# andrewli77/combinatorial-rl-tasks

Hardware: NVIDIA B200
Metric: env_steps_per_sec (higher is better)
Workload: dtype f32

## Files before the change

combinatorial_rl_tasks_b200/csrc/crl_kernels.cu:

```cuda
#include <cuda_runtime.h>

#include <atomic>
#include <stdint.h>
#include <stdio.h>
#include <string.h>

#include "../../include/crl_b200.h"
#include "crl_core.cuh"

namespace crl {

#ifndef CRL_THREADS
#define CRL_THREADS 64
#endif
constexpr int kThreads = CRL_THREADS;
constexpr unsigned kFull = 0xffffffffu;

struct KParams {
  int B, num_steps, frameskip, max_cd, seed_mode, env_offset;
  long long min_seed, max_seed;
  double thresh2;
  float r2_guard;
  double bonus_per_step;
  double beta_a, beta_b;
  float robot_keepout, zone_keepout, extent;
  unsigned flags;
  DivConst div_steps, div_cd;
  unsigned long long action_seed, step_index;
  float4* pose;
  float4* aux;
  float2* zone_xy;
  uint32_t* zone_tmax;
  uint2* cooldown;
  long long* seed;
  uint32_t* episode;
  float4* origin;
  double* counters;
  float2* next_zone_xy;
  uint32_t* next_task;
  float4* next_origin;
  long long* next_seed;
  uint32_t* next_ready;
  uint32_t* stamp;
  uint32_t* act_count;
  const uint32_t* epoch;
  uint32_t round;
  uint32_t* row_list;
  float* zone_obs_host;
  unsigned long long* result_dev;
  int32_t* goal;
  const float2* bank_zone_xy;
  const float4* bank_origin;
  const uint32_t* bank_task;
  const float4* fixed;
  uint32_t init_hi;
  uint32_t walled;
  const float2* actions;
  float4* obs;
  float* zone_obs;
  unsigned long long* result;
  float* shaped;
  const uint8_t* mask;
};

constexpr uint32_t kParBit = 0x8000u, kHiMask = 0x7fffu;

template <int TASK>
struct ZoneDim { static constexpr int Z = (TASK == CRL_TASK_TSP) ? 6 : 7; };

#ifndef CRL_REGS_N15
#define CRL_REGS_N15 112
#endif
template <int N>
struct MaxRegs { static constexpr int v = N > 8 ? CRL_REGS_N15 : 80; };

template <int N>
struct Env {
  Body b;
  float ep_return;
  int steps;
  uint32_t hi;
  float2 zone[N];
  uint32_t tmax[(N + 1) / 2];
  uint2 cd;
};

__device__ __forceinline__ uint32_t cd_get(const uint2& cd, int i) {
  const uint32_t w = i < 4 ? cd.x : cd.y;
  return (w >> (8 * (i & 3))) & 0xffu;
}
__device__ __forceinline__ void cd_set(uint2& cd, int i, uint32_t v) {
  uint32_t& w = i < 4 ? cd.x : cd.y;
  const int sh = 8 * (i & 3);
  w = (w & ~(0xffu << sh)) | (v << sh);
}
__device__ __forceinline__ uint32_t cd_dec4(uint32_t w) {
  const uint32_t nz = (((w & 0x7f7f7f7fu) + 0x7f7f7f7fu) | w) >> 7 & 0x01010101u;
  return w - nz;
}


__device__ __forceinline__ U4 draw(long long seed, uint32_t c0, uint32_t c1, uint32_t c2, uint32_t tag) {
  U4 ctr{c0, c1, c2, tag};
  return philox4x32(ctr, (uint32_t)(unsigned long long)seed, (uint32_t)((unsigned long long)seed >> 32));
}

__device__ double gamma_mt(long long seed, double a, uint32_t zone, uint32_t which) {
  const double d = a - 1.0 / 3.0, c = 1.0 / sqrt(9.0 * d);
  for (uint32_t it = 0;; ++it) {
    const U4 r0 = draw(seed, it, zone, which, kTagTask);
    const U4 r1 = draw(seed, it, zone, which + 2u, kTagTask);
    const double u1 = u01d(r0.x, r0.y), u2 = u01d(r0.z, r0.w), u3 = u01d(r1.x, r1.y);
    const double x = sqrt(-2.0 * log(u1)) * cos(2.0 * kPi * u2);
    double v = 1.0 + c * x;
    if (v <= 0.0) continue;
    v = v * v * v;
    if (log(u3) < 0.5 * x * x + d - d * v + d * log(v) || it > 64u) return d * v;
  }
}

__device__ double gamma_half_integer(long long seed, int k, uint32_t zone, uint32_t which) {
  const int m = k >> 1;
  double prod = 1.0, U = 1.0, V = 0.0;
  const int n_u = m + ((k & 1) ? 2 : 0);
  for (int j = 0; j < n_u; j += 2) {
    const U4 r = draw(seed, (uint32_t)(j >> 1), zone, which, kTagTask);
    const double ua = u01d(r.x, r.y), ub = u01d(r.z, r.w);
    if (j < m) prod *= ua; else if (j == m) U = ua; else V = ua;
    if (j + 1 < m) prod *= ub; else if (j + 1 == m) U = ub; else if (j + 1 < n_u) V = ub;
  }
  double g = -log(prod);
  if (k & 1) {
    const double c = cos(2.0 * kPi * V);
    g += -log(U) * (c * c);
  }
  return g;
}

CRL_HD int half_integer_shape(double a) {
  const double t = 2.0 * a;
  const int k = (int)t;
  return ((double)k == t && k >= 1 && k <= 16) ? k : 0;
}

__device__ double gamma_draw(long long seed, double a, uint32_t zone, uint32_t which) {
  const int k = half_integer_shape(a);
  return k ? gamma_half_integer(seed, k, zone, which) : gamma_mt(seed, a, zone, which);
}

__device__ uint32_t colour_draw(long long seed, uint32_t zone) {
  uint32_t c = 3u;
  for (uint32_t it = 0; c == 3u && it < 64u; ++it) {
    const U4 r = draw(seed, it, zone, 0u, kTagTask);
    uint32_t bits = r.x;
    for (int q = 0; q < 16 && c == 3u; ++q, bits >>= 2) c = bits & 3u;
  }
  return c == 3u ? 0u : c;
}

template <int N, bool FIXED>
__device__ void warp_layout(const KParams& p, long long seed, float2* placed, int lane) {
  const float ext = p.extent;
  constexpr int NP = (N + 2) / 2;
#pragma unroll 1
  for (uint32_t attempt = 0; attempt < 10000u; ++attempt) {
    bool ok_layout = true;
#pragma unroll 1
    for (int k = 0; k <= N && ok_layout; ++k) {
      const float keep = k == 0 ? p.robot_keepout : p.zone_keepout;
      float lo_x = -ext + keep, lo_y = lo_x, span = (ext - keep) - lo_x;
      if (FIXED && p.fixed) {
        const float4 fx = p.fixed[k];
        if (fx.w == 1.f || fx.w == 3.f) { lo_x = fx.x; lo_y = fx.y; span = 0.f; }
      }
      float4 pl[NP];
#pragma unroll
      for (int q2 = 0; q2 < NP; ++q2) pl[q2] = reinterpret_cast<const float4*>(placed)[q2];
      bool found = false;
#pragma unroll 1
      for (int base = 0; base < 100 && !found; base += 32) {
        const int j = base + lane;
        const U4 r = draw(seed, (uint32_t)(j >> 1), (uint32_t)k, attempt, kTagLayout);
        const float x = __fadd_rn(lo_x, __fmul_rn(span, u01((j & 1) ? r.z : r.x)));
        const float y = __fadd_rn(lo_y, __fmul_rn(span, u01((j & 1) ? r.w : r.y)));
        bool valid = j < 100;
#pragma unroll
        for (int q = 0; q < N; ++q) {
          const float ox = (q & 1) ? pl[q >> 1].z : pl[q >> 1].x;
          const float oy = (q & 1) ? pl[q >> 1].w : pl[q >> 1].y;
          const float need = __fadd_rn(q == 0 ? p.robot_keepout : p.zone_keepout, keep);
          const float dx = __fsub_rn(x, ox), dy = __fsub_rn(y, oy);
          const float d2 = __fmaf_rn(dy, dy, __fmul_rn(dx, dx));
          valid = valid && (q >= k || d2 >= __fmul_rn(need, need));
        }
        const unsigned m = __ballot_sync(kFull, valid);
        if (m) {
          const int wlane = __ffs(m) - 1;
          const float wx = __shfl_sync(kFull, x, wlane), wy = __shfl_sync(kFull, y, wlane);
          if (lane == 0) placed[k] = make_float2(wx, wy);
          found = true;
        }
      }
      __syncwarp();
      ok_layout = found;
    }
    if (ok_layout) return;
  }
}

__device__ __forceinline__ long long choose_seed(const KParams& p, int e, uint32_t episode, uint32_t ahead = 0u) {
  if (p.seed_mode != CRL_SEED_FIXED_RANGE) return p.seed[e] + (long long)ahead;
  const unsigned long long span = (unsigned long long)(p.max_seed - p.min_seed) + 1ull;
  const U4 r = draw((long long)(p.env_offset + e), episode + ahead, 0u, 0u, kTagSeed);
  const unsigned long long v = ((unsigned long long)r.x << 32) | r.y;
  return p.min_seed + (long long)(span ? (v % span) : v);
}

template <int TASK, int N, bool FIXED>
__device__ void warp_generate(const KParams& p, long long chosen, float2* placed, int lane,
                              uint32_t& my_draw, float& rot0) {
  my_draw = 0u;
  if (TASK == CRL_TASK_TTSP && lane < N) {
    const double ga = gamma_draw(chosen, p.beta_a, (uint32_t)lane, 0u);
    const double gb = gamma_draw(chosen, p.beta_b, (uint32_t)lane, 1u);
    const int t = (int)((ga / (ga + gb)) * (double)p.num_steps);
    my_draw = (uint32_t)min(max(t, 0), 65535);
  }
  if (TASK == CRL_TASK_CM && lane < N) my_draw = colour_draw(chosen, (uint32_t)lane);
  warp_layout<N, FIXED>(p, chosen + 1, placed, lane);
  const U4 rr = draw(chosen + 1, 0u, 0u, 0u, kTagRot);
  rot0 = __fmul_rn(6.2831855f, u01(rr.x));
  if (FIXED && p.fixed) { const float4 f0 = p.fixed[0]; if (f0.w >= 2.f) rot0 = f0.z; }
  __syncwarp();
}

constexpr uint32_t kSlotEmpty = 0u, kSlotLayoutDone = 2u, kSlotClaimed = 3u, kSlotReady = 16u;

__device__ __forceinline__ uint32_t ld_acquire_u32(const uint32_t* p) {
  uint32_t v;
  asm volatile("ld.acquire.gpu.global.u32 %0, [%1];" : "=r"(v) : "l"(p) : "memory");
  return v;
}
// ... 383 lines not shown
    } else {
      const bool v = (env.hi >> i) & 1u;
      r = v ? 1.f : 0.f; g = 1.f; b = v ? 0.f : 1.f;
    }
    float* z = row + i * Z;
    if (Z == 6) {
      reinterpret_cast<float2*>(z)[0] = make_float2(env.zone[i].x * third, env.zone[i].y * third);
      reinterpret_cast<float2*>(z)[1] = make_float2(r, g);
      reinterpret_cast<float2*>(z)[2] = make_float2(b, 0.25f);
    } else {
      z[0] = env.zone[i].x * third; z[1] = env.zone[i].y * third;
      z[2] = r; z[3] = g; z[4] = b; z[5] = 0.25f;
      if (TASK == CRL_TASK_TTSP) {
        const bool v = (env.hi >> i) & 1u;
        const int tm = (int)((env.tmax[i >> 1] >> (16 * (i & 1))) & 0xffffu);
        z[6] = v ? 1.0f : div_const((float)(tm - env.steps), p.div_steps);
      } else {
        z[6] = div_const((float)cd_get(env.cd, i), p.div_cd);
      }
    }
  }
}

template <int TASK, int N>
__device__ __forceinline__ void zone_obs_issue(const KParams& p, float* stage, int lane, int env0, int max_rows) {
  constexpr int ROW = N * ZoneDim<TASK>::Z;
  const int n_valid = max(0, min(max_rows, p.B - env0));
  const uint32_t bytes = (uint32_t)n_valid * ROW * 4u;
  float* gdst = p.zone_obs + (size_t)env0 * ROW;
  if ((bytes & 15u) == 0u) {
    asm volatile("fence.proxy.async.shared::cta;" ::: "memory");
    __syncwarp();
    if (lane == 0 && n_valid > 0) {
      const uint32_t saddr = (uint32_t)__cvta_generic_to_shared(stage);
      asm volatile("cp.async.bulk.global.shared::cta.bulk_group [%0], [%1], %2;"
                   :: "l"(gdst), "r"(saddr), "r"(bytes) : "memory");
      asm volatile("cp.async.bulk.commit_group;" ::: "memory");
    }
  } else {
    __syncwarp();
    for (int i = lane; i < n_valid * ROW; i += 32) gdst[i] = stage[i];
  }
}

template <int TASK, int N>
__device__ __forceinline__ void zone_obs_send(const KParams& p, const Env<N>& env, bool valid,
                                              float* stage, int lane, int warp_env0, bool zero_row = false) {
  constexpr int ROW = N * ZoneDim<TASK>::Z;
  if (valid) zone_row<TASK, N>(p, env, stage + lane * ROW);
  if (zero_row) {
    for (int k = 0; k < ROW; ++k) stage[lane * ROW + k] = 0.f;
  }
  zone_obs_issue<TASK, N>(p, stage, lane, warp_env0, 32);
}

template <int TASK, int N>
__device__ __noinline__ void send_rows(const KParams& p, float* out, const float* stage, unsigned mask, int lane,
                                       int warp_env0) {
  constexpr int Z = ZoneDim<TASK>::Z, ROW = N * Z;
  if (TASK == CRL_TASK_TTSP && (p.flags & CRL_STEP_HOST_PLANES)) {
    const size_t plane = (size_t)p.B * N;
    const int n_valid = max(0, min(32, p.B - warp_env0));
    float* tl = out + 6 * plane + (size_t)warp_env0 * N;
    for (int i = lane; i < n_valid * N; i += 32) tl[i] = stage[(i / N) * ROW + (i % N) * Z + 6];
    while (mask) {
      const int src = __ffs(mask) - 1;
      mask &= mask - 1u;
      const float* row = stage + src * ROW;
      float* dst = out + (size_t)(warp_env0 + src) * N;
      for (int i = lane; i < 6 * N; i += 32) dst[(size_t)(i / N) * plane + (i % N)] = row[(i % N) * Z + (i / N)];
    }
    return;
  }
  while (mask) {
    const int src = __ffs(mask) - 1;
    mask &= mask - 1u;
    float* dst = out + (size_t)(warp_env0 + src) * ROW;
    const float* row = stage + src * ROW;
    for (int i = lane; i < ROW; i += 32) dst[i] = row[i];
  }
}

template <int TASK, int N>
__device__ __forceinline__ bool zone_obs_step(const KParams& p, const Env<N>& env, float* stage, int lane, int warp_env0,
                                              unsigned changed) {
  constexpr int ROW = N * ZoneDim<TASK>::Z;
  const int n_valid = max(0, min(32, p.B - warp_env0));
  const unsigned all = n_valid >= 32 ? kFull : (1u << n_valid) - 1u;
  const unsigned m = (p.flags & CRL_STEP_ZONE_OBS_DELTA) ? changed : all;
  if ((m >> lane) & 1u) zone_row<TASK, N>(p, env, stage + lane * ROW);
  if (m != all) return false;
  zone_obs_issue<TASK, N>(p, stage, lane, warp_env0, 32);
  return true;
}

__device__ __forceinline__ void zone_obs_wait(int lane) {
  if (lane == 0) asm volatile("cp.async.bulk.wait_group.read 0;" ::: "memory");
}

constexpr int kParkedSteps = 0xffff;
__device__ void obs_rows_bulk(float4* obs, int B, float4 row0, float4 row1, bool valid, float* stage, int lane, int warp_env0);

template <int TASK, int N>
__device__ __forceinline__ void store_state_obs(const KParams& p, const Env<N>& env, int e, float c, float s,
                                                bool park = false) {
  p.pose[e] = make_float4(env.b.X, env.b.Y, env.b.phi, env.b.vx);
  p.aux[e] = make_float4(env.b.vy, env.b.w, env.ep_return,
                         __int_as_float((int)((uint32_t)(park ? kParkedSteps : env.steps) | (env.hi << 16))));
  if (TASK == CRL_TASK_CM) p.cooldown[e] = env.cd;
  const float remaining = div_const((float)(p.num_steps - env.steps), p.div_steps);
  p.obs[2 * (size_t)e] = make_float4(remaining, env.b.X * (1.0f / 3.0f), env.b.Y * (1.0f / 3.0f), c);
  p.obs[2 * (size_t)e + 1] = make_float4(s, env.b.vx * (1.0f / 1.5f), env.b.vy * (1.0f / 1.5f),
                                         env.b.w * (1.0f / 3.0f));
}

template <int TASK, int N>
__device__ __forceinline__ void store_state_obs_host(const KParams& p, const Env<N>& env, bool valid, int e, float c, float s,
                                                     float* stage, int lane, int warp_env0) {
  if (valid) {
    p.pose[e] = make_float4(env.b.X, env.b.Y, env.b.phi, env.b.vx);
    p.aux[e] = make_float4(env.b.vy, env.b.w, env.ep_return, __int_as_float((int)((uint32_t)env.steps | (env.hi << 16))));
    if (TASK == CRL_TASK_CM) p.cooldown[e] = env.cd;
  }
  const float remaining = div_const((float)(p.num_steps - env.steps), p.div_steps);
  obs_rows_bulk(p.obs, p.B, make_float4(remaining, env.b.X * (1.0f / 3.0f), env.b.Y * (1.0f / 3.0f), c),
                make_float4(s, env.b.vx * (1.0f / 1.5f), env.b.vy * (1.0f / 1.5f), env.b.w * (1.0f / 3.0f)), valid, stage, lane,
                warp_env0);
}

__device__ __noinline__ void obs_rows_bulk(float4* obs, int B, float4 row0, float4 row1, bool valid, float* stage, int lane,
                                           int warp_env0) {
  if (lane == 0) asm volatile("cp.async.bulk.wait_group.read 0;" ::: "memory");
  __syncwarp();
  if (valid) {
    float4* row = reinterpret_cast<float4*>(stage) + 2 * lane;
    row[0] = row0;
    row[1] = row1;
  }
  asm volatile("fence.proxy.async.shared::cta;" ::: "memory");
  __syncwarp();
  const int n_valid = max(0, min(32, B - warp_env0));
  if (lane == 0 && n_valid > 0) {
    const uint32_t saddr = (uint32_t)__cvta_generic_to_shared(stage);
    float4* gdst = obs + 2 * (size_t)warp_env0;
    asm volatile("cp.async.bulk.global.shared::cta.bulk_group [%0], [%1], %2;"
                 :: "l"(gdst), "r"(saddr), "r"((uint32_t)n_valid * 32u) : "memory");
    asm volatile("cp.async.bulk.commit_group;" ::: "memory");
  }
}

template <int TASK, int N>
__device__ __forceinline__ void load_env(const KParams& p, int e, Env<N>& env) {
  const float4 ps = p.pose[e];
  const float4 ax = p.aux[e];
#pragma unroll
  for (int i = 0; i < N; ++i) env.zone[i] = p.zone_xy[(size_t)i * p.B + e];
  if (TASK == CRL_TASK_TTSP) {
#pragma unroll
    for (int j = 0; j < (N + 1) / 2; ++j) env.tmax[j] = p.zone_tmax[(size_t)j * p.B + e];
  }
  if (TASK == CRL_TASK_CM) env.cd = p.cooldown[e];
  env.b.X = ps.x; env.b.Y = ps.y; env.b.phi = ps.z; env.b.vx = ps.w;
  env.b.vy = ax.x; env.b.w = ax.y; env.ep_return = ax.z;
  const uint32_t bits = (uint32_t)__float_as_int(ax.w);
  env.steps = (int)(bits & 0xffffu);
  env.hi = bits >> 16;
}

__device__ __forceinline__ double dist_np(float X, float Y, float zx, float zy) {
  const double dx = (double)zx - (double)X, dy = (double)zy - (double)Y;
  return __dsqrt_rn(__dadd_rn(__dmul_rn(dx, dx), __dmul_rn(dy, dy)));
}

__device__ __forceinline__ uint32_t chain_ticket(const KParams& p, int w, int lane) {
  uint32_t t = 0u;
  if (lane == 0 && w < (p.B + 31) / 32) t = atomicAdd(p.stamp + w, 1u);
  return t;
}

__device__ __forceinline__ void chain_wait(const KParams& p, int w, int lane, uint32_t ticket) {
  if (lane == 0 && w < (p.B + 31) / 32) {
    const uint32_t* fin = p.stamp + (p.B + 31) / 32 + w;
    uint32_t polls = 0;
    while (ld_acquire_u32(fin) != ticket) {
      __nanosleep(64);
      if (++polls > (1u << 22)) { atomicAdd(p.counters + 7, 1.0); break; }
    }
  }
  __syncwarp();
}

__device__ __forceinline__ void chain_release(const KParams& p, int w, int lane, uint32_t ticket) {
  __syncwarp();
  if (lane == 0) {
    asm volatile("cp.async.bulk.wait_group 0;" ::: "memory");
    if (w < (p.B + 31) / 32) st_release_u32(p.stamp + (p.B + 31) / 32 + w, ticket + 1u);
  }
}

template <int TASK, int N, bool EXT, bool FIXED = false>
__global__ void __maxnreg__(MaxRegs<N>::v) step_kernel(const __grid_constant__ KParams p) {
  constexpr int ROW = N * ZoneDim<TASK>::Z;
  extern __shared__ __align__(128) float smem[];
  const int lane = threadIdx.x & 31, warp = threadIdx.x >> 5;
  const int e = blockIdx.x * kThreads + threadIdx.x;
  const int warp_env0 = blockIdx.x * kThreads + warp * 32;
  const bool valid = e < p.B;
  float* stage = smem + warp * (32 * ROW);
  uint32_t ticket = 0u;
  const bool ticketed = (p.flags & (CRL_STEP_CHAINED | CRL_STEP_CHAIN_START)) != 0u;
  if (ticketed) {
    ticket = chain_ticket(p, warp_env0 >> 5, lane);
    asm volatile("griddepcontrol.launch_dependents;" :: "r"(ticket) : "memory");
  } else {
    asm volatile("griddepcontrol.launch_dependents;" ::: "memory");
  }
  if (p.flags & CRL_STEP_CHAINED) {
    chain_wait(p, warp_env0 >> 5, lane, ticket);
  } else {
    asm volatile("griddepcontrol.wait;" ::: "memory");
  }

  uint32_t act_base = 0u;
  uint32_t* act_cnt = nullptr;
  if (!p.actions && (p.flags & CRL_STEP_ACTION_COUNTER) && lane == 0 && warp_env0 < p.B) {
    act_cnt = p.act_count + (warp_env0 >> 5);
    act_base = ld_relaxed_u32(act_cnt);
  }
  Env<N> env;
  float2 act = make_float2(0.f, 0.f);
  if (valid) load_env<TASK, N>(p, e, env);
  if (!p.actions && (p.flags & CRL_STEP_ACTION_COUNTER)) {
    if (act_cnt) *act_cnt = act_base + 1u;
    act_base = __shfl_sync(kFull, act_base, 0);
  }
  if (valid) {
    if (p.actions) {
      act = p.actions[e];
    } else {
      const unsigned ge = (unsigned)(p.env_offset + e);
      const unsigned long long si = p.step_index + act_base;
      U4 ctr{ge, (uint32_t)si, (uint32_t)(si >> 32), kTagAction};
      const U4 r = philox4x32(ctr, (uint32_t)p.action_seed, (uint32_t)(p.action_seed >> 32));
      act = make_float2(2.f * u01(r.x) - 1.f, 2.f * u01(r.y) - 1.f);
    }
  } else {
    env.b = Body{0.f, 0.f, 0.f, 0.f, 0.f, 0.f};
    env.ep_return = 0.f; env.steps = 0; env.hi = 0u; env.cd = make_uint2(0u, 0u);
#pragma unroll
    for (int i = 0; i < N; ++i) env.zone[i] = make_float2(1e9f, 1e9f);
#pragma unroll
    for (int j = 0; j < (N + 1) / 2; ++j) env.tmax[j] = 0xffffffffu;
  }

  const bool parked = EXT && (p.flags & CRL_STEP_WAIT) && valid && env.steps == kParkedSteps;
  const bool live = valid && !parked;
  const bool revive = EXT && parked && (p.flags & CRL_STEP_AUTO_RESET);
  const bool goals = EXT && (p.flags & CRL_STEP_GOALS);
  int goal_zone = -1;
  float gzx = 0.f, gzy = 0.f;
  double dist_before = 0.0;
  Body old_b = env.b;
  bool reached = false, park_now = false;
  if (goals && live) {
    goal_zone = p.goal[e];
    if (goal_zone >= 0) {
#pragma unroll
      for (int j = 0; j < N; ++j) if (j == goal_zone) { gzx = env.zone[j].x; gzy = env.zone[j].y; }
      dist_before = dist_np(env.b.X, env.b.Y, gzx, gzy);
    }
  }
  int fired_out = -1;
  __shared__ unsigned s_rows_mask[kThreads / 32];
  const bool some_rows = p.zone_obs_host || (p.flags & CRL_STEP_ZONE_OBS_DELTA);
  if (some_rows && lane == 0) s_rows_mask[warp] = 0u;
  bool fresh = false;
  if (!(p.flags & CRL_STEP_PHYSICS_ONLY)) {
    bool row_changed = TASK == CRL_TASK_TTSP && !(p.flags & CRL_STEP_HOST_PLANES);
    if (TASK == CRL_TASK_CM) {
      row_changed = (env.cd.x | env.cd.y) != 0u;
      env.cd.x = cd_dec4(env.cd.x); env.cd.y = cd_dec4(env.cd.y);
    }
    uint32_t cand = 0u;
#pragma unroll
    for (int i = 0; i < N; ++i)
      if (near_zone(env.b.X, env.b.Y, env.zone[i].x, env.zone[i].y, p.r2_guard)) cand |= 1u << i;
    if (TASK == CRL_TASK_CM) {
      if (cand) {
#pragma unroll
        for (int i = 0; i < N; ++i) if (cd_get(env.cd, i) != 0u) cand &= ~(1u << i);
      }
    } else {
      cand &= ~env.hi;
    }
    int fired = -1;
    while (cand) {
      const int i = __ffs(cand) - 1;
      cand &= cand - 1u;
      float zx = 0.f, zy = 0.f;
#pragma unroll
      for (int j = 0; j < N; ++j) if (j == i) { zx = env.zone[j].x; zy = env.zone[j].y; }
      if (inside_zone(env.b.X, env.b.Y, zx, zy, p.thresh2)) { fired = i; break; }
    }
    int event = 0;
    if (fired >= 0) {
      if (TASK == CRL_TASK_CM) {
        const int old_dist = hamming(env.hi, N);
        const uint32_t col = (env.hi >> (2 * fired)) & 3u;
        const uint32_t nxt = col == 2u ? 0u : col + 1u;
        env.hi = (env.hi & ~(3u << (2 * fired))) | (nxt << (2 * fired));
        cd_set(env.cd, fired, (uint32_t)p.max_cd);
        event = old_dist - hamming(env.hi, N);
      } else {
        env.hi |= 1u << fired;
        event = 1;
      }
    }
    bool goal;
    if (TASK == CRL_TASK_CM) {
      constexpr uint32_t kOnes = ((1u << (2 * N)) - 1u) & 0x55555555u;
      const uint32_t col = env.hi & kHiMask;
      goal = col == 0u || col == kOnes || col == 2u * kOnes;
    } else {
      goal = (env.hi & kHiMask) == ((1u << N) - 1u);
    }
    bool done = false;
    float reward = (float)event;
    if (goal) {
      reward = (float)((double)event + (double)(p.num_steps - env.steps) * p.bonus_per_step);
      done = true;
    }
    env.steps = min(env.steps + 1, kParkedSteps - 1);
    if (env.steps >= p.num_steps) done = true;
    if (TASK == CRL_TASK_TTSP && !done) {
#pragma unroll
      for (int i = 0; i < N; ++i) {
        const int tm = (int)((env.tmax[i >> 1] >> (16 * (i & 1))) & 0xffffu);
        if (!((env.hi >> i) & 1u) && env.steps >= tm) done = true;
      }
    }
    env.ep_return += reward;
    done = done && live;
    goal = goal && live;
    if (EXT) {
      fired_out = fired;
      reached = goals && fired >= 0 && fired == goal_zone;
      park_now = (p.flags & CRL_STEP_WAIT) && done && !(p.flags & CRL_STEP_AUTO_RESET);
      if (parked) { reward = 0.f; event = 0; }
    }
    if (p.flags & (CRL_STEP_TRACK_ROWS | CRL_STEP_ZONE_OBS_DELTA)) {
      const bool ch = (live && (row_changed || fired >= 0 || (done && (p.flags & CRL_STEP_AUTO_RESET)))) || parked;
      const unsigned cm = __ballot_sync(kFull, ch);
      if (some_rows && lane == 0) s_rows_mask[warp] = cm;
      if ((p.flags & CRL_STEP_TRACK_ROWS) && cm && lane == 0) atomicAdd(p.row_list, __popc(cm));
    }
    bool res_moved = false;
    if (valid) {
      const bool need_next = goals && live && (reached || done || goal_zone < 0);
      const unsigned long long word = (unsigned long long)__float_as_uint(reward) |
          ((unsigned long long)((done || parked) ? 1u : 0u) << 32) | ((unsigned long long)(goal ? 1u : 0u) << 40) |
          ((unsigned long long)(uint8_t)(int8_t)event << 48) | ((unsigned long long)(need_next ? 1u : 0u) << 56);
      if (p.result_dev) {
        const unsigned long long prev = p.result_dev[e];
        p.result_dev[e] = word;
        if (prev != word) { p.result[e] = word; res_moved = true; }
      } else {
        p.result[e] = word;
      }
      if (EXT && goals && live && need_next && goal_zone >= 0) p.goal[e] = -1;
    }
    if (p.result_dev) {
      const unsigned mm = __ballot_sync(kFull, res_moved);
      if (mm && lane == 0) atomicAdd(p.row_list + 1, (uint32_t)__popc(mm));
    }
    const unsigned dm = __ballot_sync(kFull, done);
    const unsigned rm = EXT ? __ballot_sync(kFull, done || revive) : dm;
    if (rm) {
      float ret = done ? env.ep_return : 0.f;
      float len = done ? (float)env.steps : 0.f;
      const unsigned gm = __ballot_sync(kFull, goal);
#pragma unroll
      for (int o = 16; o > 0; o >>= 1) {
        ret += __shfl_xor_sync(kFull, ret, o);
        len += __shfl_xor_sync(kFull, len, o);
      }
      if (lane == 0 && dm) {
        atomicAdd(p.counters + 0, (double)ret);
        atomicAdd(p.counters + 1, (double)__popc(dm));
        atomicAdd(p.counters + 2, (double)__popc(gm));
        atomicAdd(p.counters + 3, (double)len);
      }
      if (p.flags & CRL_STEP_AUTO_RESET) {
        fresh = done || revive;
        const uint32_t par_in = env.hi >> 15;
        bool served = false;
        if (fresh) served = reset_from_slot<TASK, N>(p, e, env);
        const unsigned sm = __ballot_sync(kFull, served);
        if (lane == 0 && sm) atomicAdd(p.counters + 4, (double)__popc(sm));
        const unsigned left = rm & ~sm;
        if (left) {
          Env<N> next = env;
          warp_reset<TASK, N, FIXED>(p, left, lane, e, reinterpret_cast<float2*>(stage), par_in, next);
          env = next;
        }
      }
    }
  }
  float c, s;
  if (!EXT) {
    unsigned rows = 0u;
    if (some_rows) {
      __syncwarp();
      rows = s_rows_mask[warp];
    }
    if (!(p.flags & CRL_STEP_NO_ZONE_OBS) && zone_obs_step<TASK, N>(p, env, stage, lane, warp_env0, rows) && !p.zone_obs_host)
      rows = 0u;
    if (rows || p.zone_obs_host) {
      __syncwarp();
      send_rows<TASK, N>(p, p.zone_obs_host ? p.zone_obs_host : p.zone_obs, stage, rows, lane, warp_env0);
    }
    if (fresh) {
      sincosf(env.b.phi, &s, &c);
    } else {
      substeps(env.b, act.x, act.y, p.frameskip, c, s);
      env.b.phi = wrap_pi(env.b.phi);
    }
    if (p.zone_obs_host) {
      store_state_obs_host<TASK, N>(p, env, valid, e, c, s, stage, lane, warp_env0);
    } else if (valid) {
      store_state_obs<TASK, N>(p, env, e, c, s);
    }
  } else {
    if (!(p.flags & CRL_STEP_NO_ZONE_OBS))
      zone_obs_send<TASK, N>(p, env, live || revive, stage, lane, warp_env0, parked && !revive);
    if (p.zone_obs_host) send_rows<TASK, N>(p, p.zone_obs_host, stage, s_rows_mask[warp], lane, warp_env0);
    Body pb = fresh ? old_b : env.b;
    if (p.walled) substeps<CRL_CONTACT_MODEL, true>(pb, act.x, act.y, p.frameskip, c, s, p.extent);
    else substeps(pb, act.x, act.y, p.frameskip, c, s);
    if (fresh) {
      sincosf(env.b.phi, &s, &c);
    } else {
      env.b = pb;
      env.b.phi = wrap_pi(env.b.phi);
    }
    if (goals && live) {
      double shaped = 0.0;
      if (goal_zone >= 0 && !reached) {
        shaped = dist_before - dist_np(pb.X, pb.Y, gzx, gzy);
        if (TASK == CRL_TASK_CM && fired_out >= 0) shaped -= 1.0;
      }
      p.shaped[e] = (float)shaped;
    }
    if (parked && goals) p.shaped[e] = 0.f;
    if (parked && !revive) {
      p.obs[2 * (size_t)e] = make_float4(0.f, 0.f, 0.f, 0.f);
      p.obs[2 * (size_t)e + 1] = make_float4(0.f, 0.f, 0.f, 0.f);
    } else if (valid) {
      store_state_obs<TASK, N>(p, env, e, c, s, park_now);
    }
  }
  if (ticketed) {
    chain_release(p, warp_env0 >> 5, lane, ticket);
  } else {
    zone_obs_wait(lane);
  }
}

template <int TASK, int N>
__global__ void __launch_bounds__(kThreads) reset_kernel(const __grid_constant__ KParams p) {
  constexpr int ROW = N * ZoneDim<TASK>::Z;
  extern __shared__ __align__(128) float smem[];
  const int lane = threadIdx.x & 31, warp = threadIdx.x >> 5;
  const int e = blockIdx.x * kThreads + threadIdx.x;
  const int warp_env0 = blockIdx.x * kThreads + warp * 32;
  const bool valid = e < p.B;
  float* stage = smem + warp * (32 * ROW);
  Env<N> env;
  if (valid) load_env<TASK, N>(p, e, env);
  const bool want = valid && (p.mask == nullptr || p.mask[e] != 0);
  const unsigned m = __ballot_sync(kFull, want);
  if (m) warp_reset<TASK, N, true, true>(p, m, lane, e, reinterpret_cast<float2*>(stage), 0u, env);
  float c = 1.f, s = 0.f;
  if (valid) sincosf(env.b.phi, &s, &c);
  zone_obs_send<TASK, N>(p, env, valid, stage, lane, warp_env0);
  if (want) store_state_obs<TASK, N>(p, env, e, c, s);
  zone_obs_wait(lane);
}

struct LayoutParams {
  const double* xy0; const double* rot0; const double* zone_xy;
  const int32_t* zone_max_steps; const int32_t* colours; const int32_t* env_ids; int n;
};

template <int TASK, int N>
__global__ void reset_from_layout_kernel(const KParams p, const LayoutParams L) {
  constexpr int ROW = N * ZoneDim<TASK>::Z;
  const int i = blockIdx.x * blockDim.x + threadIdx.x;
  if (i >= L.n) return;
  const int e = L.env_ids ? L.env_ids[i] : i;
  if (e < 0 || e >= p.B) return;
  Env<N> env;
  const float rot0 = (float)L.rot0[i];
  env.b = Body{(float)L.xy0[2 * i], (float)L.xy0[2 * i + 1], wrap_pi(rot0), 0.f, 0.f, 0.f};
  env.ep_return = 0.f; env.steps = 0; env.hi = TASK == CRL_TASK_CM ? 0u : p.init_hi; env.cd = make_uint2(0u, 0u);
#pragma unroll
  for (int j = 0; j < (N + 1) / 2; ++j) env.tmax[j] = 0u;
#pragma unroll
  for (int z = 0; z < N; ++z) {
    env.zone[z] = make_float2((float)L.zone_xy[((size_t)i * N + z) * 2], (float)L.zone_xy[((size_t)i * N + z) * 2 + 1]);
    p.zone_xy[(size_t)z * p.B + e] = env.zone[z];
    if (TASK == CRL_TASK_TTSP) {
      const uint32_t t = (uint32_t)min(max(L.zone_max_steps[(size_t)i * N + z], 0), 65535);
      env.tmax[z >> 1] |= t << (16 * (z & 1));
    }
    if (TASK == CRL_TASK_CM) env.hi |= ((uint32_t)L.colours[(size_t)i * N + z] & 3u) << (2 * z);
  }
  if (TASK == CRL_TASK_TTSP) {
#pragma unroll
    for (int j = 0; j < (N + 1) / 2; ++j) p.zone_tmax[(size_t)j * p.B + e] = env.tmax[j];
  }
  const uint32_t episode = p.episode[e] + 1u;
  p.episode[e] = episode;
  if (p.goal) p.goal[e] = -1;
  p.origin[e] = make_float4(env.b.X, env.b.Y, rot0, 0.f);
  p.pose[e] = make_float4(env.b.X, env.b.Y, env.b.phi, 0.f);
  p.aux[e] = make_float4(0.f, 0.f, 0.f, __int_as_float((int)((env.hi << 16) | ((episode & 1u) << 31))));
  if (TASK == CRL_TASK_CM) p.cooldown[e] = env.cd;
  float c, s;
  sincosf(env.b.phi, &s, &c);
  p.obs[2 * (size_t)e] = make_float4(1.0f, env.b.X * (1.0f / 3.0f), env.b.Y * (1.0f / 3.0f), c);
  p.obs[2 * (size_t)e + 1] = make_float4(s, 0.f, 0.f, 0.f);
  __align__(16) float row[ROW];
  zone_row<TASK, N>(p, env, row);
  float* g = p.zone_obs + (size_t)e * ROW;
#pragma unroll
  for (int k = 0; k < ROW; ++k) g[k] = row[k];
}

__global__ void set_qpos_qvel_kernel(const KParams p, const double* qpos, const double* qvel,
                                     const int32_t* env_ids, int n) {
  const int i = blockIdx.x * blockDim.x + threadIdx.x;
  if (i >= n) return;
  const int e = env_ids ? env_ids[i] : i;
  if (e < 0 || e >= p.B) return;
  const float4 o = p.origin[e];
  const double c0 = cos((double)o.z), s0 = sin((double)o.z);
// ... 219 lines not shown
  for (int i = 0; i < used; ++i)
    if (slots[i].d == d && slots[i].lo == n_lo && slots[i].hi == n_hi) return slots[i].k;
  const DivConst k = make_div_const(d, n_lo, n_hi);
  if (used < 8) slots[used++] = Slot{d, n_lo, n_hi, k};
  return k;
}

static int fill_params(const CrlConfig* c, const CrlState* st, const CrlOut* out, KParams& p) {
  int rc = check_config(c);
  if (rc) return rc;
  if (!st || !st->pose || !st->aux || !st->zone_xy || !st->seed || !st->episode || !st->origin || !st->counters)
    return CRL_ERR_NULL;
  if (c->task == CRL_TASK_TTSP && !st->zone_tmax) return CRL_ERR_NULL;
  if (c->task == CRL_TASK_CM && !st->cooldown) return CRL_ERR_NULL;
  if (!aligned16(st->pose) || !aligned16(st->aux) || !aligned16(st->zone_xy) || !aligned16(st->origin))
    return CRL_ERR_ALIGN;
  memset(&p, 0, sizeof(p));
  p.B = c->num_envs; p.num_steps = c->num_steps; p.frameskip = c->frameskip; p.max_cd = c->max_cooldown;
  p.seed_mode = c->seed_mode; p.env_offset = c->env_offset; p.min_seed = c->min_seed; p.max_seed = c->max_seed;
  p.thresh2 = sqrt_threshold(c->zone_size);
  p.r2_guard = (float)(c->zone_size * c->zone_size * 1.001 + 1e-5);
  p.bonus_per_step = c->time_saved_reward;
  p.beta_a = c->beta_a; p.beta_b = c->beta_b;
  p.div_steps = cached_div_const(c->num_steps, -65535, 65535);
  p.div_cd = cached_div_const(c->max_cooldown > 0 ? c->max_cooldown : 1, 0, 255);
  if (!p.div_steps.exact || !p.div_cd.exact) return CRL_ERR_CONFIG;
  p.robot_keepout = (float)c->robot_keepout; p.zone_keepout = (float)c->zone_keepout; p.extent = (float)c->extent;
  p.pose = reinterpret_cast<float4*>(st->pose); p.aux = reinterpret_cast<float4*>(st->aux);
  p.zone_xy = reinterpret_cast<float2*>(st->zone_xy); p.zone_tmax = st->zone_tmax;
  p.cooldown = reinterpret_cast<uint2*>(st->cooldown);
  p.seed = reinterpret_cast<long long*>(st->seed); p.episode = st->episode;
  p.origin = reinterpret_cast<float4*>(st->origin); p.counters = st->counters;
  if (st->next_ready) {
    if (!st->next_zone_xy || !st->next_origin || !st->next_seed || (c->task != CRL_TASK_TSP && !st->next_task))
      return CRL_ERR_NULL;
    if (!aligned16(st->next_origin) || !aligned16(st->next_zone_xy)) return CRL_ERR_ALIGN;
    p.next_zone_xy = reinterpret_cast<float2*>(st->next_zone_xy); p.next_task = st->next_task;
    p.next_origin = reinterpret_cast<float4*>(st->next_origin);
    p.next_seed = reinterpret_cast<long long*>(st->next_seed); p.next_ready = st->next_ready;
  }
  if (st->fixed_layout) {
    if (!aligned16(st->fixed_layout)) return CRL_ERR_ALIGN;
    p.fixed = reinterpret_cast<const float4*>(st->fixed_layout);
  }
  p.init_hi = c->task == CRL_TASK_CM ? 0u : c->initial_visited;
  p.walled = c->walled;
  p.stamp = st->stamp;
  p.act_count = st->stamp ? st->stamp + 2 * (size_t)((c->num_envs + 31) / 32) : nullptr;
  p.epoch = st->prefetch_epoch;
  if (p.next_ready && !p.epoch) return CRL_ERR_NULL;
  p.row_list = st->row_list;
  p.goal = st->goal;
  if (st->bank_zone_xy || st->bank_origin || st->bank_task) {
    if (!st->bank_zone_xy || !st->bank_origin || (c->task != CRL_TASK_TSP && !st->bank_task)) return CRL_ERR_NULL;
    if (c->max_seed < c->min_seed) return CRL_ERR_CONFIG;
    if (!aligned16(st->bank_origin) || (reinterpret_cast<uintptr_t>(st->bank_zone_xy) & 7u)) return CRL_ERR_ALIGN;
    p.bank_zone_xy = reinterpret_cast<const float2*>(st->bank_zone_xy);
    p.bank_origin = reinterpret_cast<const float4*>(st->bank_origin);
    p.bank_task = st->bank_task;
  }
  if (out) {
    if (!out->obs || !out->result) return CRL_ERR_NULL;
    if (!aligned16(out->obs) || !aligned16(out->zone_obs)) return CRL_ERR_ALIGN;
    p.obs = reinterpret_cast<float4*>(out->obs); p.zone_obs = out->zone_obs;
    p.result = reinterpret_cast<unsigned long long*>(out->result);
    p.shaped = out->shaped_reward;
  }
  return CRL_OK;
}

static int launch_status() { return cudaGetLastError() == cudaSuccess ? CRL_OK : CRL_ERR_LAUNCH; }

#define CRL_DISPATCH(task, n, CALL)                                              \
  do {                                                                           \
    if ((task) == CRL_TASK_TSP && (n) == 15) { CALL(CRL_TASK_TSP, 15); }         \
    else if ((task) == CRL_TASK_TSP && (n) == 5) { CALL(CRL_TASK_TSP, 5); }      \
    else if ((task) == CRL_TASK_TTSP && (n) == 15) { CALL(CRL_TASK_TTSP, 15); }  \
    else if ((task) == CRL_TASK_TTSP && (n) == 5) { CALL(CRL_TASK_TTSP, 5); }    \
    else if ((task) == CRL_TASK_CM && (n) == 6) { CALL(CRL_TASK_CM, 6); }        \
    else return CRL_ERR_UNSUPPORTED;                                             \
  } while (0)

template <int T, int NN>
static void (*pick_step_kernel(bool ext, bool fixed))(const KParams) {
  if (fixed) {
    if constexpr (T == CRL_TASK_TSP && NN == 15) return ext ? step_kernel<T, NN, true, true> : step_kernel<T, NN, false, true>;
    else return nullptr;
  }
  return ext ? step_kernel<T, NN, true> : step_kernel<T, NN, false>;
}

static int set_smem(void (*kernel)(const KParams), size_t bytes) {
  static void (*done_for[32])(const KParams) = {nullptr};
  if (bytes <= 48 * 1024) return CRL_OK;
  for (int i = 0; i < 32; ++i) {
    if (done_for[i] == kernel) return CRL_OK;
    if (done_for[i] == nullptr) {
      if (cudaFuncSetAttribute(kernel, cudaFuncAttributeMaxDynamicSharedMemorySize, (int)bytes) != cudaSuccess)
        return CRL_ERR_DEVICE;
      done_for[i] = kernel;
      return CRL_OK;
    }
  }
  return CRL_ERR_DEVICE;
}

}

using namespace crl;

extern "C" {

int crl_abi_version(void) { return CRL_ABI_VERSION; }

const char* crl_strerror(int code) {
  switch (code) {
    case CRL_OK: return "ok";
    case CRL_ERR_NULL: return "a required pointer is NULL";
    case CRL_ERR_CONFIG: return "CrlConfig out of range";
    case CRL_ERR_ALIGN: return "a float4 plane is not 16-byte aligned";
    case CRL_ERR_UNSUPPORTED: return "no kernel compiled for this (task, num_zones)";
    case CRL_ERR_LAUNCH: return "CUDA launch failed";
    case CRL_ERR_DEVICE: return "CUDA device/runtime error";
    default: return "unknown error";
  }
}

int crl_plane_bytes(const CrlConfig* c, int64_t* out_bytes, int32_t n) {
  int rc = check_config(c);
  if (rc) return rc;
  if (!out_bytes) return CRL_ERR_NULL;
  if (n < 0) return CRL_ERR_CONFIG;
  int64_t o[CRL_NUM_PLANES];
  const int64_t B = c->num_envs, N = c->num_zones, Z = zone_dim(c->task);
  o[0] = 16 * B; o[1] = 16 * B; o[2] = 8 * N * B;
  o[3] = c->task == CRL_TASK_TTSP ? 4 * ((N + 1) / 2) * B : 0;
  o[4] = c->task == CRL_TASK_CM ? 8 * B : 0;
  o[5] = 8 * B; o[6] = 4 * B; o[7] = 16 * B; o[8] = 8 * 8;
  o[9] = 2 * 8 * N * B;
  o[10] = 2 * (c->task == CRL_TASK_TTSP ? 4 * ((N + 1) / 2) * B : (c->task == CRL_TASK_CM ? 4 * B : 0));
  o[11] = 2 * 16 * B; o[12] = 2 * 8 * B; o[13] = 2 * 4 * B;
  o[14] = 32 * B; o[15] = 4 * N * Z * B; o[16] = 8 * B;
  o[17] = 3 * 4 * ((B + 31) / 32);
  o[18] = 16 * (1 + 2 * B);
  o[19] = 16;
  o[20] = 4 * B;
  o[21] = 4 * B;
  o[22] = 16;
  for (int i = 0; i < n && i < CRL_NUM_PLANES; ++i) out_bytes[i] = o[i];
  return CRL_OK;
}

int crl_step_bytes(const CrlConfig* c, int64_t* rd, int64_t* wr) {
  int rc = check_config(c);
  if (rc) return rc;
  if (!rd || !wr) return CRL_ERR_NULL;
  const int64_t N = c->num_zones, Z = zone_dim(c->task);
  int64_t r = 8  + 32  + 8 * N, w = 32 + 8  + 32  + 4 * N * Z;
  if (c->task == CRL_TASK_TTSP) r += 4 * ((N + 1) / 2);
  if (c->task == CRL_TASK_CM) { r += 8; w += 8; }
  *rd = r; *wr = w;
  return CRL_OK;
}

static int step_launch(const CrlConfig* c, const CrlState* st, const float* actions, const CrlOut* out,
                       uint32_t flags, uint64_t action_seed, uint64_t step_index, float* zone_obs_host, void* stream,
                       CrlResult* result_dev = nullptr) {
  KParams p;
  if (!out) return CRL_ERR_NULL;
  int rc = fill_params(c, st, out, p);
  if (rc) return rc;
  p.zone_obs_host = zone_obs_host;
  p.result_dev = reinterpret_cast<unsigned long long*>(result_dev);
  if (result_dev && (!zone_obs_host || !p.row_list)) return CRL_ERR_CONFIG;
  if (actions && (reinterpret_cast<uintptr_t>(actions) & 7u)) return CRL_ERR_ALIGN;
  p.actions = reinterpret_cast<const float2*>(actions);
  p.flags = flags; p.action_seed = action_seed; p.step_index = step_index;
  const bool ticketed = (flags & (CRL_STEP_CHAINED | CRL_STEP_CHAIN_START)) != 0u;
  if (ticketed && !p.stamp) return CRL_ERR_NULL;
  if ((flags & CRL_STEP_TRACK_ROWS) && !p.row_list) return CRL_ERR_NULL;
  if ((flags & CRL_STEP_GOALS) && (!p.goal || !p.shaped)) return CRL_ERR_NULL;
  if ((flags & CRL_STEP_ACTION_COUNTER) && !p.act_count) return CRL_ERR_NULL;
  if (!(flags & CRL_STEP_NO_ZONE_OBS) && !p.zone_obs) return CRL_ERR_NULL;
  if ((flags & CRL_STEP_NO_ZONE_OBS) && (zone_obs_host || (flags & CRL_STEP_TRACK_ROWS))) return CRL_ERR_CONFIG;
  if ((flags & CRL_STEP_HOST_PLANES) && (!zone_obs_host || c->task != CRL_TASK_TTSP)) return CRL_ERR_CONFIG;
  const bool ext = (flags & (CRL_STEP_GOALS | CRL_STEP_WAIT)) != 0u || c->walled != 0u;
  if ((flags & CRL_STEP_ZONE_OBS_DELTA) && (ext || zone_obs_host || (flags & CRL_STEP_NO_ZONE_OBS))) return CRL_ERR_CONFIG;
  if (c->task == CRL_TASK_TTSP) p.flags &= ~CRL_STEP_ZONE_OBS_DELTA;
  static std::atomic<void*> last_chained_stream{reinterpret_cast<void*>(-1)};
  const bool after_chained = last_chained_stream.load(std::memory_order_relaxed) == stream;
  const bool programmatic = (flags & CRL_STEP_CHAINED) || !after_chained;
  last_chained_stream.store((flags & CRL_STEP_CHAINED) ? stream : reinterpret_cast<void*>(-1), std::memory_order_relaxed);
  const int blocks = (p.B + kThreads - 1) / kThreads;
  cudaStream_t s = static_cast<cudaStream_t>(stream);
#define CRL_CALL_STEP(T, NN)                                                        \
  {                                                                                 \
    const size_t sm = (size_t)kThreads * NN * ZoneDim<T>::Z * 4;                    \
    void (*kern)(const KParams) = pick_step_kernel<T, NN>(ext, p.fixed != nullptr); \
    if (!kern) return CRL_ERR_UNSUPPORTED;                                          \
    rc = set_smem(kern, sm);                                                        \
    if (rc) return rc;                                                              \
    cudaLaunchConfig_t lc = {};                                                     \
    lc.gridDim = dim3(blocks); lc.blockDim = dim3(kThreads);                        \
    lc.dynamicSmemBytes = sm; lc.stream = s;                                        \
    cudaLaunchAttribute at[1];                                                      \
    at[0].id = cudaLaunchAttributeProgrammaticStreamSerialization;                  \
    at[0].val.programmaticStreamSerializationAllowed = 1;                           \
    lc.attrs = at; lc.numAttrs = programmatic ? 1 : 0;                              \
    if (cudaLaunchKernelEx(&lc, kern, p) != cudaSuccess) {                          \
      (void)cudaGetLastError();                                                     \
      return CRL_ERR_LAUNCH;                                                        \
    }                                                                               \
  }
  CRL_DISPATCH(c->task, c->num_zones, CRL_CALL_STEP);
  return launch_status();
}

int crl_step(const CrlConfig* c, const CrlState* st, const float* actions, const CrlOut* out,
             uint32_t flags, uint64_t action_seed, uint64_t step_index, void* stream) {
  return step_launch(c, st, actions, out, flags, action_seed, step_index, nullptr, stream);
}

int crl_reset(const CrlConfig* c, const CrlState* st, const CrlOut* out, const uint8_t* mask, void* stream) {
  KParams p;
  if (!out || !out->zone_obs) return CRL_ERR_NULL;
  int rc = fill_params(c, st, out, p);
  if (rc) return rc;
  p.mask = mask;
  const int blocks = (p.B + kThreads - 1) / kThreads;
  cudaStream_t s = static_cast<cudaStream_t>(stream);
#define CRL_CALL_RESET(T, NN)                                                       \
  {                                                                                 \
    const size_t sm = (size_t)kThreads * NN * ZoneDim<T>::Z * 4;                    \
    rc = set_smem(reset_kernel<T, NN>, sm);                                         \
    if (rc) return rc;                                                              \
    reset_kernel<T, NN><<<blocks, kThreads, sm, s>>>(p);                            \
  }
  CRL_DISPATCH(c->task, c->num_zones, CRL_CALL_RESET);
  return launch_status();
}

int crl_reset_from_layout(const CrlConfig* c, const CrlState* st, const CrlOut* out, const CrlLayoutIn* lay,
                          const int32_t* env_ids, int32_t n, void* stream) {
  KParams p;
  if (!out || !out->zone_obs || !lay || !lay->xy0 || !lay->rot0 || !lay->zone_xy) return CRL_ERR_NULL;
  int rc = fill_params(c, st, out, p);
  if (rc) return rc;
  if (c->task == CRL_TASK_TTSP && !lay->zone_max_steps) return CRL_ERR_NULL;
  if (c->task == CRL_TASK_CM && !lay->colours) return CRL_ERR_NULL;
  if (n < 0 || n > c->num_envs) return CRL_ERR_CONFIG;
  if (n == 0) return CRL_OK;
  LayoutParams L{lay->xy0, lay->rot0, lay->zone_xy, lay->zone_max_steps, lay->colours, env_ids, n};
  cudaStream_t s = static_cast<cudaStream_t>(stream);
#define CRL_CALL_LAYOUT(T, NN) { reset_from_layout_kernel<T, NN><<<(n + 127) / 128, 128, 0, s>>>(p, L); }
  CRL_DISPATCH(c->task, c->num_zones, CRL_CALL_LAYOUT);
  return launch_status();
}

int crl_prefetch_layouts(const CrlConfig* c, const CrlState* st, int32_t warps_per_sm, uint32_t round, void* stream) {
  KParams p;
  int rc = fill_params(c, st, nullptr, p);
  if (rc) return rc;
  if (!p.next_ready || !st->prefetch_work || !p.epoch) return CRL_ERR_NULL;
  if (round > 0xffffff00u) return CRL_ERR_CONFIG;
  p.round = round;
  if (!aligned16(st->prefetch_work)) return CRL_ERR_ALIGN;
  if (warps_per_sm <= 0) warps_per_sm = 2;
  if (warps_per_sm > 32) warps_per_sm = 32;
  WorkItem* work = reinterpret_cast<WorkItem*>(st->prefetch_work);
  cudaStream_t s = static_cast<cudaStream_t>(stream);
  if (cudaMemsetAsync(work, 0, sizeof(WorkHeader), s) != cudaSuccess) return CRL_ERR_DEVICE;
  const int blocks_0 = min((p.B + 63) / 64, 148 * 8);
#define CRL_CALL_PREFETCH_0(T, NN) { prefetch_scan_kernel<NN><<<blocks_0, 64, 0, s>>>(p, work); }
  CRL_DISPATCH(c->task, c->num_zones, CRL_CALL_PREFETCH_0);
  const int blocks_a = min((2 * p.B + 31) / 32, 148 * warps_per_sm);
  const uint32_t done_state = c->task == CRL_TASK_TSP ? kSlotReady + round : kSlotLayoutDone;
#define CRL_CALL_PREFETCH_A(T, NN) { prefetch_layout_kernel<NN><<<blocks_a, 32, 0, s>>>(p, work, done_state); }
  CRL_DISPATCH(c->task, c->num_zones, CRL_CALL_PREFETCH_A);
  rc = launch_status();
  if (rc || c->task == CRL_TASK_TSP) return rc;
  const int blocks_b = min((2 * p.B + 1) / 2, 148 * 4);
// ... 213 lines not shown
```

Before: 18.89 billion.

## Add lean stage-free step kernel with in-place delta zone-obs writes

Adds a LEAN step_kernel variant, chosen when zone-obs delta or no-zone-obs mode is set without ext or host rows. It drops the per-warp shared-memory staging, loads zone coordinates on demand instead of holding them in registers, caps registers at 64, and writes only the changed zone-obs fields straight to global memory. The goal is higher occupancy and less smem/bulk-copy traffic, at the cost of extra scattered global loads and stores.

```diff
diff --git a/combinatorial_rl_tasks_b200/csrc/crl_kernels.cu b/combinatorial_rl_tasks_b200/csrc/crl_kernels.cu
--- a/combinatorial_rl_tasks_b200/csrc/crl_kernels.cu
+++ b/combinatorial_rl_tasks_b200/csrc/crl_kernels.cu
@@ -73,6 +73,9 @@
 #endif
 template <int N>
 struct MaxRegs { static constexpr int v = N > 8 ? CRL_REGS_N15 : 80; };
+#ifndef CRL_REGS_LEAN
+#define CRL_REGS_LEAN 64
+#endif
 
 template <int N>
 struct Env {
@@ -158,6 +161,8 @@
   return c == 3u ? 0u : c;
 }
 
+template <int N>
+constexpr int kPlacedFloats = 4 * ((N + 2) / 2);
 template <int N, bool FIXED>
 __device__ void warp_layout(const KParams& p, long long seed, float2* placed, int lane) {
   const float ext = p.extent;
@@ -707,16 +712,23 @@
 }
 
 template <int TASK, int N>
-__device__ __forceinline__ bool zone_obs_step(const KParams& p, const Env<N>& env, float* stage, int lane, int warp_env0,
-                                              unsigned changed) {
-  constexpr int ROW = N * ZoneDim<TASK>::Z;
-  const int n_valid = max(0, min(32, p.B - warp_env0));
-  const unsigned all = n_valid >= 32 ? kFull : (1u << n_valid) - 1u;
-  const unsigned m = (p.flags & CRL_STEP_ZONE_OBS_DELTA) ? changed : all;
-  if ((m >> lane) & 1u) zone_row<TASK, N>(p, env, stage + lane * ROW);
-  if (m != all) return false;
-  zone_obs_issue<TASK, N>(p, stage, lane, warp_env0, 32);
-  return true;
+__device__ __forceinline__ void zone_row_event(const KParams& p, const Env<N>& env, int e, int fired, bool cd_moved) {
+  constexpr int Z = ZoneDim<TASK>::Z;
+  float* row = p.zone_obs + (size_t)e * (N * Z);
+  if (TASK == CRL_TASK_CM) {
+    if (fired >= 0) {
+      const uint32_t c = (env.hi >> (2 * fired)) & 3u;
+      float* z = row + fired * Z;
+      z[2] = c == 2u ? 1.f : 0.f; z[3] = c == 1u ? 1.f : 0.f; z[4] = c == 0u ? 1.f : 0.f;
+    }
+    if (cd_moved) {
+#pragma unroll
+      for (int i = 0; i < N; ++i) row[i * Z + 6] = div_const((float)cd_get(env.cd, i), p.div_cd);
+    }
+  } else if (fired >= 0) {
+    float* z = row + fired * Z;
+    z[2] = 1.f; z[4] = 0.f;
+  }
 }
 
 __device__ __forceinline__ void zone_obs_wait(int lane) {
@@ -774,12 +786,14 @@
   }
 }
 
-template <int TASK, int N>
+template <int TASK, int N, bool ZONES = true>
 __device__ __forceinline__ void load_env(const KParams& p, int e, Env<N>& env) {
   const float4 ps = p.pose[e];
   const float4 ax = p.aux[e];
-#pragma unroll
-  for (int i = 0; i < N; ++i) env.zone[i] = p.zone_xy[(size_t)i * p.B + e];
+  if (ZONES) {
+#pragma unroll
+    for (int i = 0; i < N; ++i) env.zone[i] = p.zone_xy[(size_t)i * p.B + e];
+  }
   if (TASK == CRL_TASK_TTSP) {
 #pragma unroll
     for (int j = 0; j < (N + 1) / 2; ++j) env.tmax[j] = p.zone_tmax[(size_t)j * p.B + e];
@@ -823,15 +837,16 @@
   }
 }
 
-template <int TASK, int N, bool EXT, bool FIXED = false>
-__global__ void __maxnreg__(MaxRegs<N>::v) step_kernel(const __grid_constant__ KParams p) {
+template <int TASK, int N, bool EXT, bool FIXED = false, bool LEAN = false>
+__global__ void __maxnreg__(LEAN ? CRL_REGS_LEAN : MaxRegs<N>::v) step_kernel(const __grid_constant__ KParams p) {
+  static_assert(!(LEAN && EXT), "the stage-free step has no EXT variant");
   constexpr int ROW = N * ZoneDim<TASK>::Z;
   extern __shared__ __align__(128) float smem[];
   const int lane = threadIdx.x & 31, warp = threadIdx.x >> 5;
   const int e = blockIdx.x * kThreads + threadIdx.x;
   const int warp_env0 = blockIdx.x * kThreads + warp * 32;
   const bool valid = e < p.B;
-  float* stage = smem + warp * (32 * ROW);
+  float* stage = smem + warp * (LEAN ? kPlacedFloats<N> : 32 * ROW);
   uint32_t ticket = 0u;
   const bool ticketed = (p.flags & (CRL_STEP_CHAINED | CRL_STEP_CHAIN_START)) != 0u;
   if (ticketed) {
@@ -854,7 +869,17 @@
   }
   Env<N> env;
   float2 act = make_float2(0.f, 0.f);
-  if (valid) load_env<TASK, N>(p, e, env);
+  uint32_t near = 0u;
+  if (valid) {
+    load_env<TASK, N, !LEAN>(p, e, env);
+    if (LEAN) {
+#pragma unroll
+      for (int i = 0; i < N; ++i) {
+        const float2 z = p.zone_xy[(size_t)i * p.B + e];
+        if (near_zone(env.b.X, env.b.Y, z.x, z.y, p.r2_guard)) near |= 1u << i;
+      }
+    }
+  }
   if (!p.actions && (p.flags & CRL_STEP_ACTION_COUNTER)) {
     if (act_cnt) *act_cnt = act_base + 1u;
     act_base = __shfl_sync(kFull, act_base, 0);
@@ -897,8 +922,9 @@
   }
   int fired_out = -1;
   __shared__ unsigned s_rows_mask[kThreads / 32];
-  const bool some_rows = p.zone_obs_host || (p.flags & CRL_STEP_ZONE_OBS_DELTA);
+  const bool some_rows = !LEAN && p.zone_obs_host;
   if (some_rows && lane == 0) s_rows_mask[warp] = 0u;
+  const bool delta = LEAN && TASK != CRL_TASK_TTSP && (p.flags & CRL_STEP_ZONE_OBS_DELTA);
   bool fresh = false;
   if (!(p.flags & CRL_STEP_PHYSICS_ONLY)) {
     bool row_changed = TASK == CRL_TASK_TTSP && !(p.flags & CRL_STEP_HOST_PLANES);
@@ -906,10 +932,12 @@
       row_changed = (env.cd.x | env.cd.y) != 0u;
       env.cd.x = cd_dec4(env.cd.x); env.cd.y = cd_dec4(env.cd.y);
     }
-    uint32_t cand = 0u;
-#pragma unroll
-    for (int i = 0; i < N; ++i)
-      if (near_zone(env.b.X, env.b.Y, env.zone[i].x, env.zone[i].y, p.r2_guard)) cand |= 1u << i;
+    uint32_t cand = near;
+    if (!LEAN) {
+#pragma unroll
+      for (int i = 0; i < N; ++i)
+        if (near_zone(env.b.X, env.b.Y, env.zone[i].x, env.zone[i].y, p.r2_guard)) cand |= 1u << i;
+    }
     if (TASK == CRL_TASK_CM) {
       if (cand) {
 #pragma unroll
@@ -923,8 +951,13 @@
       const int i = __ffs(cand) - 1;
       cand &= cand - 1u;
       float zx = 0.f, zy = 0.f;
-#pragma unroll
-      for (int j = 0; j < N; ++j) if (j == i) { zx = env.zone[j].x; zy = env.zone[j].y; }
+      if (LEAN) {
+        const float2 z = p.zone_xy[(size_t)i * p.B + e];
+        zx = z.x; zy = z.y;
+      } else {
+#pragma unroll
+        for (int j = 0; j < N; ++j) if (j == i) { zx = env.zone[j].x; zy = env.zone[j].y; }
+      }
       if (inside_zone(env.b.X, env.b.Y, zx, zy, p.thresh2)) { fired = i; break; }
     }
     int event = 0;
@@ -973,12 +1006,13 @@
       park_now = (p.flags & CRL_STEP_WAIT) && done && !(p.flags & CRL_STEP_AUTO_RESET);
       if (parked) { reward = 0.f; event = 0; }
     }
-    if (p.flags & (CRL_STEP_TRACK_ROWS | CRL_STEP_ZONE_OBS_DELTA)) {
+    if (p.flags & (CRL_STEP_TRACK_ROWS | CRL_STEP_HOST_PLANES)) {
       const bool ch = (live && (row_changed || fired >= 0 || (done && (p.flags & CRL_STEP_AUTO_RESET)))) || parked;
       const unsigned cm = __ballot_sync(kFull, ch);
       if (some_rows && lane == 0) s_rows_mask[warp] = cm;
       if ((p.flags & CRL_STEP_TRACK_ROWS) && cm && lane == 0) atomicAdd(p.row_list, __popc(cm));
     }
+    if (delta && valid) zone_row_event<TASK, N>(p, env, e, fired, row_changed || fired >= 0);
     bool res_moved = false;
     if (valid) {
       const bool need_next = goals && live && (reached || done || goal_zone < 0);
@@ -1019,11 +1053,20 @@
         fresh = done || revive;
         const uint32_t par_in = env.hi >> 15;
         bool served = false;
-        if (fresh) served = reset_from_slot<TASK, N>(p, e, env);
+        if (fresh) {
+          served = reset_from_slot<TASK, N>(p, e, env);
+          if (delta && served) zone_row<TASK, N>(p, env, p.zone_obs + (size_t)e * ROW);
+        }
         const unsigned sm = __ballot_sync(kFull, served);
         if (lane == 0 && sm) atomicAdd(p.counters + 4, (double)__popc(sm));
         const unsigned left = rm & ~sm;
-        if (left) {
+        if (left && LEAN) {
+          Env<N> next;
+          next.b = env.b; next.ep_return = env.ep_return; next.steps = env.steps; next.hi = env.hi; next.cd = env.cd;
+          warp_reset<TASK, N, FIXED>(p, left, lane, e, reinterpret_cast<float2*>(stage), par_in, next);
+          env.b = next.b; env.ep_return = next.ep_return; env.steps = next.steps; env.hi = next.hi; env.cd = next.cd;
+          if (delta && ((left >> lane) & 1u)) zone_row<TASK, N>(p, next, p.zone_obs + (size_t)e * ROW);
+        } else if (left) {
           Env<N> next = env;
           warp_reset<TASK, N, FIXED>(p, left, lane, e, reinterpret_cast<float2*>(stage), par_in, next);
           env = next;
@@ -1033,16 +1076,12 @@
   }
   float c, s;
   if (!EXT) {
-    unsigned rows = 0u;
-    if (some_rows) {
-      __syncwarp();
-      rows = s_rows_mask[warp];
-    }
-    if (!(p.flags & CRL_STEP_NO_ZONE_OBS) && zone_obs_step<TASK, N>(p, env, stage, lane, warp_env0, rows) && !p.zone_obs_host)
-      rows = 0u;
-    if (rows || p.zone_obs_host) {
-      __syncwarp();
-      send_rows<TASK, N>(p, p.zone_obs_host ? p.zone_obs_host : p.zone_obs, stage, rows, lane, warp_env0);
+    if (!LEAN) {
+      if (!(p.flags & CRL_STEP_NO_ZONE_OBS)) zone_obs_send<TASK, N>(p, env, valid, stage, lane, warp_env0);
+      if (some_rows) {
+        __syncwarp();
+        send_rows<TASK, N>(p, p.zone_obs_host, stage, s_rows_mask[warp], lane, warp_env0);
+      }
     }
     if (fresh) {
       sincosf(env.b.phi, &s, &c);
@@ -1086,7 +1125,7 @@
   }
   if (ticketed) {
     chain_release(p, warp_env0 >> 5, lane, ticket);
-  } else {
+  } else if (!LEAN) {
     zone_obs_wait(lane);
   }
 }
@@ -1472,12 +1511,13 @@
   } while (0)
 
 template <int T, int NN>
-static void (*pick_step_kernel(bool ext, bool fixed))(const KParams) {
+static void (*pick_step_kernel(bool ext, bool fixed, bool lean))(const KParams) {
   if (fixed) {
-    if constexpr (T == CRL_TASK_TSP && NN == 15) return ext ? step_kernel<T, NN, true, true> : step_kernel<T, NN, false, true>;
+    if constexpr (T == CRL_TASK_TSP && NN == 15)
+      return ext ? step_kernel<T, NN, true, true> : lean ? step_kernel<T, NN, false, true, true> : step_kernel<T, NN, false, true>;
     else return nullptr;
   }
-  return ext ? step_kernel<T, NN, true> : step_kernel<T, NN, false>;
+  return ext ? step_kernel<T, NN, true> : lean ? step_kernel<T, NN, false, false, true> : step_kernel<T, NN, false>;
 }
 
 static int set_smem(void (*kernel)(const KParams), size_t bytes) {
@@ -1577,6 +1617,7 @@
   const bool ext = (flags & (CRL_STEP_GOALS | CRL_STEP_WAIT)) != 0u || c->walled != 0u;
   if ((flags & CRL_STEP_ZONE_OBS_DELTA) && (ext || zone_obs_host || (flags & CRL_STEP_NO_ZONE_OBS))) return CRL_ERR_CONFIG;
   if (c->task == CRL_TASK_TTSP) p.flags &= ~CRL_STEP_ZONE_OBS_DELTA;
+  const bool lean = (p.flags & (CRL_STEP_ZONE_OBS_DELTA | CRL_STEP_NO_ZONE_OBS)) && !ext && !zone_obs_host;
   static std::atomic<void*> last_chained_stream{reinterpret_cast<void*>(-1)};
   const bool after_chained = last_chained_stream.load(std::memory_order_relaxed) == stream;
   const bool programmatic = (flags & CRL_STEP_CHAINED) || !after_chained;
@@ -1585,8 +1626,9 @@
   cudaStream_t s = static_cast<cudaStream_t>(stream);
 #define CRL_CALL_STEP(T, NN)                                                        \
   {                                                                                 \
-    const size_t sm = (size_t)kThreads * NN * ZoneDim<T>::Z * 4;                    \
-    void (*kern)(const KParams) = pick_step_kernel<T, NN>(ext, p.fixed != nullptr); \
+    const size_t sm = lean ? (size_t)(kThreads / 32) * kPlacedFloats<NN> * 4        \
+                           : (size_t)kThreads * NN * ZoneDim<T>::Z * 4;             \
+    void (*kern)(const KParams) = pick_step_kernel<T, NN>(ext, p.fixed != nullptr, lean); \
     if (!kern) return CRL_ERR_UNSUPPORTED;                                          \
     rc = set_smem(kern, sm);                                                        \
     if (rc) return rc;                                                              \
```

After: 24.56 billion, median of 6. +30.0%, better.
